# aubin-tchoi/shot-fpfh

Measured on AMD Instinct MI355X. Metric: descriptors/sec (SHOT+FPFH) on 1M-pt cloud, higher is better.
Workload: dtype f64

## Files before the change

### shot_fpfh_amd/csrc/common.h

```cpp
#pragma once
#include <hip/hip_runtime.h>

#include <cstdarg>
#include <cstdint>
#include <cstdio>
#include <cstring>
#include <map>
#include <atomic>
#include <tuple>
#include <string>
#include <vector>

#include "../../include/shotfpfh.h"

extern std::atomic<unsigned long long> g_sf_sync_count;
static inline hipError_t sf_counted_stream_sync(hipStream_t s)
{
    g_sf_sync_count.fetch_add(1, std::memory_order_relaxed);
    return hipStreamSynchronize(s);
}
#define hipStreamSynchronize(s) sf_counted_stream_sync(s)

#define SF_WAVE 64
constexpr double SF_DBL_MAX = 1.7976931348623157e308;
// ... 12 lines not shown
#define SF_HIP_NULL(call)                                                                             \
    do {                                                                                              \
        hipError_t e_ = (call);                                                                       \
        if (e_ != hipSuccess) {                                                                       \
            sf_set_error("%s failed: %s (%s:%d)", #call, hipGetErrorString(e_), __FILE__, __LINE__); \
            return nullptr;                                                                           \
        }                                                                                             \
    } while (0)

#define SF_CHECK(expr)      \
    do {                    \
        int rc_ = (expr);   \
        if (rc_ != SF_OK) return rc_; \
    } while (0)

struct sf_prof_entry {
    int64_t launches = 0;
    std::vector<std::pair<hipEvent_t, hipEvent_t>> pending;
    double total_ms = 0.0;
};

struct sf_graph {
    hipGraph_t graph = nullptr;
    hipGraphExec_t exec = nullptr;
    std::vector<void *> held;
};

struct sf_ctx {
    int device = 0;
    hipStream_t stream = nullptr;
    hipStream_t streams[2] = {nullptr, nullptr};
    hipEvent_t join_event = nullptr;
    hipEvent_t mark_event = nullptr;
    bool profiling = false;
    std::string prof_only;
    std::map<std::string, sf_prof_entry> prof;
    std::vector<hipEvent_t> event_pool;
    void *comm = nullptr;
    int nranks = 1, rank = 0;
    bool collective_stats = false;
    void *scratch = nullptr;
    size_t scratch_bytes = 0;
    void *pinned = nullptr;
    double *shot_coef = nullptr;
    volatile int *dev_flag = nullptr;
    std::multimap<size_t, void *> pool_free;
    std::map<void *, size_t> pool_size;
    size_t pool_cached = 0;
    sf_graph *capture = nullptr;
};

int sf_pool_alloc(sf_ctx *ctx, size_t bytes, void **out);
void sf_pool_release(sf_ctx *ctx, void *p);
void sf_pool_trim(sf_ctx *ctx);
template <typename T>
static inline int sf_palloc(sf_ctx *ctx, T **out, size_t count)
{
    void *p = nullptr;
    int rc = sf_pool_alloc(ctx, (count ? count : 1) * sizeof(T), &p);
    *out = (T *)p;
    return rc;
}

struct sf_pool_guard {
    sf_ctx *ctx;
    std::vector<void *> held;
// ... 53 lines not shown
            ctx->prof[name].launches++;
        }
    }
};

#define SF_LAUNCH(ctx, name, kernel, grid, block, ...)                                   \
    do {                                                                                 \
        sf_launch_timer t_((ctx), (name));                                               \
        hipLaunchKernelGGL(kernel, (grid), (block), 0, (ctx)->stream, __VA_ARGS__);      \
    } while (0);                                                                         \
    SF_HIP(hipGetLastError())

struct sf_cloud {
    int64_t n = 0;
    double *xyz_orig = nullptr;
    double *nrm_orig = nullptr;
    int32_t *zperm = nullptr;
    int32_t *perm_int = nullptr;
    bool bbox_known = false;
    double bbox_lo[3] = {0, 0, 0}, bbox_hi[3] = {0, 0, 0};
    uint64_t grid_gen = 0;
    double cell = 0.0;
    double inv_cell = 0.0;
    double lo[3] = {0, 0, 0};
    int dim[3] = {1, 1, 1};
    int xsub = 1;
    int64_t ncell = 0;
    int32_t *cell_start = nullptr;
    int32_t *perm = nullptr;
    int32_t *inv_perm = nullptr;
    bool inv_perm_valid = false;
    double *xs = nullptr, *ys = nullptr, *zs = nullptr;
    double *rec = nullptr;
    bool normals_sorted = false;
    double nrm_max2 = -1.0;
    int64_t pop_begin = 0, pop_end = 0;
    double *z_orig = nullptr;
    std::vector<double> z_host;
    int32_t *cell_count = nullptr;
    int64_t cell_count_cap = 0;
    bool count_dirty = false;
    std::vector<int64_t> layer_first;
    std::map<std::pair<double, bool>, std::pair<double, int64_t>> list_stats;
    struct search_record {
        int64_t total = 0, n_overflow = 0, ovf_total = 0, cap = 0, hist[5] = {0, 0, 0, 0, 0};
        int32_t max_count = 0, max_count_all = 0;
        bool folded = false;
    };
    typedef std::tuple<double, double, int, int64_t, int64_t> search_key;
    std::map<search_key, search_record> search_records;
};

struct sf_nbrs {
    int64_t m = 0;
    double radius = 0.0;
    int64_t total = 0;
    int64_t max_count = 0;
    int64_t max_count_all = 0;
    bool view = false;
    bool self = false;
    int64_t self_begin = 0;
    double *qx = nullptr, *qy = nullptr, *qz = nullptr;
    int32_t *qrow = nullptr;
    int32_t *count = nullptr;
    int64_t *offset = nullptr;
    int32_t *idx = nullptr;
    int32_t *idx_ovf = nullptr;
    int64_t cap = 0;
    int64_t n_overflow = 0;
    int64_t hist[5] = {0, 0, 0, 0, 0};
    bool planned = false;
    int main_chunks = 4;
    int tail_limit = 0x7fffffff;
    int32_t *tail_sel = nullptr;
    int64_t n_tail = 0;
    int32_t *mid_sel = nullptr;
    int64_t n_mid = 0;
    int64_t view_first = 0;
    uint64_t grid_gen = 0;
};

static inline void sf_nbrs_stamp(sf_nbrs *nb, const sf_cloud *c) { nb->grid_gen = c->grid_gen; }
static inline int sf_nbrs_on_grid(const sf_nbrs *nb, const sf_cloud *c, const char *who)
{
// ... 58 lines not shown
```

### shot_fpfh_amd/csrc/context.hip

```cpp
#include "common.h"

static thread_local char g_err[1024] = "";

void sf_set_error(const char *fmt, ...)
{
    va_list ap;
    va_start(ap, fmt);
    vsnprintf(g_err, sizeof(g_err), fmt, ap);
    va_end(ap);
}

extern "C" const char *sf_last_error(void) { return g_err; }
#ifndef SF_BUILD_ID
#define SF_BUILD_ID "unknown"
#endif
extern "C" const char *sf_version(void) { return "shotfpfh-gfx950 0.3 build " SF_BUILD_ID; }

extern "C" int sf_device_count(void)
{
    int n = 0;
    if (hipGetDeviceCount(&n) != hipSuccess) return 0;
    return n;
}

extern "C" sf_ctx *sf_create(int device)
{
    int n = 0;
    hipError_t e = hipGetDeviceCount(&n);
    if (e != hipSuccess || n <= 0) {
        sf_set_error("no HIP device available (%s); libshotfpfh has no CPU fallback",
                     e == hipSuccess ? "device count 0" : hipGetErrorString(e));
        return nullptr;
    }
    if (device < 0 || device >= n) {
        sf_set_error("device %d out of range (0..%d)", device, n - 1);
        return nullptr;
    }
    SF_HIP_NULL(hipSetDevice(device));
    sf_ctx *ctx = new sf_ctx();
    ctx->device = device;
    e = hipStreamCreateWithFlags(&ctx->streams[0], hipStreamNonBlocking);
    int prio_lo = 0, prio_hi = 0;
    (void)hipDeviceGetStreamPriorityRange(&prio_lo, &prio_hi);
    if (e == hipSuccess) e = hipStreamCreateWithPriority(&ctx->streams[1], hipStreamNonBlocking, prio_hi);
    if (e == hipSuccess) e = hipEventCreateWithFlags(&ctx->join_event, hipEventDisableTiming);
    if (e == hipSuccess) e = hipEventCreateWithFlags(&ctx->mark_event, hipEventDisableTiming);
    if (e != hipSuccess) {
        sf_set_error("hipStreamCreate failed: %s", hipGetErrorString(e));
        delete ctx;
        return nullptr;
    }
    ctx->stream = ctx->streams[0];
    void *flag = nullptr;
    if (hipHostMalloc(&flag, 64, hipHostMallocMapped) != hipSuccess) {
        sf_set_error("hipHostMalloc failed");
        delete ctx;
        return nullptr;
    }
    memset(flag, 0, 64);
    ctx->dev_flag = (volatile int *)flag;
    return ctx;
}

int sf_ctx_check_flag(sf_ctx *ctx)
{
    if (!ctx->dev_flag || !*ctx->dev_flag) return SF_OK;
    const int bits = *ctx->dev_flag;
    *ctx->dev_flag = 0;
    sf_set_error("an index array passed to the library holds values out of range:%s%s (the offending elements were skipped)",
                 bits & SF_FLAG_ROWS_GATHER ? " sf_rows_gather's row selection" : "",
                 bits & SF_FLAG_VOXEL_ORDER ? " sf_voxels_select's visiting order" : "");
    return SF_ERR_ARG;
}

extern "C" void sf_destroy(sf_ctx *ctx)
{
    if (!ctx) return;
    (void)hipSetDevice(ctx->device);
    (void)hipStreamSynchronize(ctx->streams[0]);
    (void)hipStreamSynchronize(ctx->streams[1]);
    ctx->stream = ctx->streams[0];
    sf_comm_destroy(ctx);
    for (auto &kv : ctx->prof)
        for (auto &p : kv.second.pending) {
            ctx->event_pool.push_back(p.first);
            ctx->event_pool.push_back(p.second);
        }
    for (hipEvent_t ev : ctx->event_pool) (void)hipEventDestroy(ev);
    if (ctx->scratch) (void)hipFree(ctx->scratch);
    if (ctx->pinned) (void)hipHostFree(ctx->pinned);
    if (ctx->shot_coef) (void)hipFree(ctx->shot_coef);
    if (ctx->dev_flag) (void)hipHostFree((void *)ctx->dev_flag);
    sf_pool_trim(ctx);
    for (auto &kv : ctx->pool_size) (void)hipFree(kv.first);
    (void)hipEventDestroy(ctx->join_event);
    (void)hipStreamDestroy(ctx->streams[0]);
    (void)hipStreamDestroy(ctx->streams[1]);
    delete ctx;
}

extern "C" int sf_sync(sf_ctx *ctx)
{
    if (!ctx) { sf_set_error("null ctx"); return SF_ERR_ARG; }
    SF_HIP(hipStreamSynchronize(ctx->streams[0]));
    SF_HIP(hipStreamSynchronize(ctx->streams[1]));
    return sf_ctx_check_flag(ctx);
}

extern "C" int sf_fork(sf_ctx *ctx)
{
    if (!ctx) { sf_set_error("null ctx"); return SF_ERR_ARG; }
    if (ctx->stream != ctx->streams[0]) { sf_set_error("sf_fork: already forked"); return SF_ERR_STATE; }
    SF_HIP(hipEventRecord(ctx->join_event, ctx->streams[0]));
    SF_HIP(hipStreamWaitEvent(ctx->streams[1], ctx->join_event, 0));
    ctx->stream = ctx->streams[1];
    return SF_OK;
}

extern "C" int sf_switch(sf_ctx *ctx, int side)
{
    if (!ctx || side < 0 || side > 1) { sf_set_error("sf_switch: bad argument"); return SF_ERR_ARG; }
    ctx->stream = ctx->streams[side];
    return SF_OK;
}

extern "C" int sf_join(sf_ctx *ctx)
{
    if (!ctx) { sf_set_error("null ctx"); return SF_ERR_ARG; }
    SF_HIP(hipEventRecord(ctx->join_event, ctx->streams[1]));
    SF_HIP(hipStreamWaitEvent(ctx->streams[0], ctx->join_event, 0));
    ctx->stream = ctx->streams[0];
    return SF_OK;
}

extern "C" int sf_mark(sf_ctx *ctx)
{
    if (!ctx) { sf_set_error("null ctx"); return SF_ERR_ARG; }
    SF_HIP(hipEventRecord(ctx->mark_event, ctx->stream));
    return SF_OK;
}

extern "C" int sf_wait_mark(sf_ctx *ctx)
{
    if (!ctx) { sf_set_error("null ctx"); return SF_ERR_ARG; }
    SF_HIP(hipStreamWaitEvent(ctx->stream, ctx->mark_event, 0));
    return SF_OK;
}

extern "C" void *sf_stream(sf_ctx *ctx) { return ctx ? (void *)ctx->stream : nullptr; }

std::atomic<unsigned long long> g_sf_sync_count{0};
extern "C" unsigned long long sf_sync_count(void) { return g_sf_sync_count.load(std::memory_order_relaxed); }

extern "C" int sf_graph_begin(sf_ctx *ctx)
{
    if (!ctx) { sf_set_error("null ctx"); return SF_ERR_ARG; }
    if (ctx->capture) { sf_set_error("sf_graph_begin: already capturing"); return SF_ERR_STATE; }
    if (ctx->stream != ctx->streams[0]) { sf_set_error("sf_graph_begin: forked (sf_join first)"); return SF_ERR_STATE; }
    if (ctx->profiling) { sf_set_error("sf_graph_begin: launch timers are on (sf_profile(0) first)"); return SF_ERR_STATE; }
    SF_HIP(hipSetDevice(ctx->device));
    SF_HIP(hipStreamSynchronize(ctx->streams[0]));
    SF_HIP(hipStreamSynchronize(ctx->streams[1]));
    SF_HIP(hipStreamBeginCapture(ctx->streams[0], hipStreamCaptureModeThreadLocal));
    ctx->capture = new sf_graph();
    return SF_OK;
}

extern "C" sf_graph *sf_graph_end(sf_ctx *ctx)
{
    if (!ctx || !ctx->capture) { sf_set_error("sf_graph_end: not capturing"); return nullptr; }
    sf_graph *g = ctx->capture;
    ctx->capture = nullptr;
    ctx->stream = ctx->streams[0];
    hipError_t e = hipStreamEndCapture(ctx->streams[0], &g->graph);
    if (e == hipSuccess && g->graph) e = hipGraphInstantiate(&g->exec, g->graph, nullptr, nullptr, 0);
    if (e != hipSuccess || !g->exec) {
        sf_set_error("sf_graph_end: the step could not be captured (%s)", hipGetErrorString(e));
        (void)hipGetLastError();
        sf_graph_free(ctx, g);
        return nullptr;
    }
    return g;
}

extern "C" int sf_graph_launch(sf_ctx *ctx, sf_graph *g)
{
    if (!ctx || !g || !g->exec) { sf_set_error("sf_graph_launch: bad argument"); return SF_ERR_ARG; }
    if (ctx->capture) { sf_set_error("sf_graph_launch: capturing"); return SF_ERR_STATE; }
    SF_HIP(hipGraphLaunch(g->exec, ctx->streams[0]));
    return SF_OK;
}

extern "C" void sf_graph_free(sf_ctx *ctx, sf_graph *g)
{
    if (!g) return;
// ... 212 lines not shown
```

### shot_fpfh_amd/csrc/fpfh.hip

```cpp
#include <algorithm>
#include <cmath>
#include <cstring>

#include "common.h"
#include "device_util.h"

namespace {

#include "fpfh_mc.h"

template <typename CT, int LPR, int NP, int NCH>
__global__ __launch_bounds__(256) void k_fpfh(const double *__restrict__ rec, const int64_t *__restrict__ offset,
                                              const int32_t *__restrict__ cnt, const int32_t *__restrict__ idx,
                                              int64_t nbrs_begin,
                                              const int32_t *__restrict__ kp_pos, int64_t m, int nb3, int stride,
                                              const CT *__restrict__ counts, unsigned table_bytes,
                                              const int32_t *__restrict__ kk, double *__restrict__ out)
{
    constexpr int BPP = 16 / (int)sizeof(CT);
    constexpr int RPI = 64 / LPR;
    const int lane = threadIdx.x & 63;
    const int64_t q = sf_uniform64(sf_xcd_block() * 4 + (threadIdx.x >> 6));
    if (q >= m) return;
    const int64_t i = kp_pos ? (int64_t)kp_pos[q] : nbrs_begin + q;
// ... 464 lines not shown
}

static int fpfh_run(sf_ctx *ctx, sf_cloud *c, sf_nbrs *nb, sf_spfh *sp, const int64_t *kp_idx, int64_t m, double *out, int flags,
                    double *cov);

extern "C" int sf_fpfh(sf_ctx *ctx, sf_cloud *c, sf_nbrs *nb, sf_spfh *sp, const int64_t *kp_idx, int64_t m, double *out,
                       int flags)
{
    return fpfh_run(ctx, c, nb, sp, kp_idx, m, out, flags, nullptr);
}

extern "C" int sf_fpfh_moments(sf_ctx *ctx, sf_cloud *c, sf_nbrs *nb, sf_spfh *sp, int64_t m, double *out, double *cov_dev, int flags)
{
    if (!cov_dev) { sf_set_error("sf_fpfh_moments: null cov"); return SF_ERR_ARG; }
    if (nb && sp && !fpfh_mc_carries_moments(nb, sp)) {
        sf_set_error("sf_fpfh_moments: these lists / this table do not take a K7 form that carries the frame moments");
        return SF_ERR_UNSUPPORTED;
    }
    return fpfh_run(ctx, c, nb, sp, nullptr, m, out, flags, cov_dev);
}

static int fpfh_run(sf_ctx *ctx, sf_cloud *c, sf_nbrs *nb, sf_spfh *sp, const int64_t *kp_idx, int64_t m, double *out, int flags,
                    double *cov)
{
    if (!ctx || !c || !nb || !sp || !out || m < 0) { sf_set_error("sf_fpfh: bad argument"); return SF_ERR_ARG; }
    if (!nb->self) { sf_set_error("sf_fpfh: needs a sf_radius_search_self result"); return SF_ERR_ARG; }
    SF_CHECK(sf_nbrs_on_grid(nb, c, "sf_fpfh"));
    if (!kp_idx && m != nb->m) { sf_set_error("sf_fpfh: m must equal the query count when kp_idx is NULL"); return SF_ERR_ARG; }
    if (kp_idx && !(nb->self_begin == 0 && nb->m == c->n)) {
        sf_set_error("sf_fpfh: keypoints by index need neighbour lists of the whole cloud");
        return SF_ERR_ARG;
    }
    SF_HIP(hipSetDevice(ctx->device));
    sf_pool_guard tmp(ctx);
    int32_t *pos = nullptr;
    if (kp_idx && m) {
        const int64_t *src = kp_idx;
        int64_t *dkp = nullptr;
        int *dbad = nullptr;
        if (!(flags & SF_IN_DEVICE)) {
            SF_CHECK(tmp.alloc(&dkp, (size_t)m));
            SF_HIP(hipMemcpyAsync(dkp, kp_idx, (size_t)m * sizeof(int64_t), hipMemcpyHostToDevice, ctx->stream));
            src = dkp;
        }
        SF_CHECK(tmp.alloc(&pos, (size_t)m));
        SF_CHECK(tmp.alloc(&dbad, 1));
        SF_HIP(hipMemsetAsync(dbad, 0, sizeof(int), ctx->stream));
        SF_CHECK(sf_cloud_ensure_inv_perm(ctx, c));
        SF_LAUNCH(ctx, "k7_map_positions", k_map_positions, dim3((unsigned)sf_div_up(m, 256)), dim3(256), src,
                  c->inv_perm, m, c->n, pos, dbad);
        int bad = 0;
        SF_HIP(hipMemcpyAsync(&bad, dbad, sizeof(int), hipMemcpyDeviceToHost, ctx->stream));
        SF_HIP(hipStreamSynchronize(ctx->stream));
        if (bad) {
            sf_set_error("sf_fpfh: keypoint index out of range for a cloud of %lld points", (long long)c->n);
            return SF_ERR_ARG;
        }
    }
    const int64_t tot = m * sp->nb3;
    double *dout = out, *owned = nullptr;
    if (!(flags & SF_OUT_DEVICE)) {
        SF_CHECK(tmp.alloc(&owned, (size_t)tot));
        dout = owned;
    }
    int rc = SF_OK;
    if (m && sp->n_bins > SF_FAST_FPFH_BINS && sp->elem_bytes != 1) {
// ... 15 lines not shown
```

### shot_fpfh_amd/csrc/grid.hip

```cpp
#include <rocprim/device/device_radix_sort.hpp>
#include <rocprim/device/device_reduce.hpp>
#include <rocprim/device/device_scan.hpp>
#include <rocprim/iterator/transform_iterator.hpp>

#include <algorithm>
#include <cmath>

#include <cstring>

#include "common.h"
#include "device_util.h"

#ifndef SF_SORT_BITS
#define SF_SORT_BITS 10
#endif
#ifndef SF_SORT_BLOCK
#define SF_SORT_BLOCK 1024
#endif
#ifndef SF_SORT_ITEMS
#define SF_SORT_ITEMS 6
#endif
using sf_onesweep = rocprim::radix_sort_onesweep_config<rocprim::kernel_config<SF_SORT_BLOCK, SF_SORT_ITEMS>, rocprim::kernel_config<SF_SORT_BLOCK, SF_SORT_ITEMS>,
                                                        SF_SORT_BITS, rocprim::block_radix_rank_algorithm::match>;
using sf_sort_config = rocprim::radix_sort_config<rocprim::default_config, rocprim::default_config, sf_onesweep, 65536>;
// ... 77 lines not shown
    if (i >= n) return;
    const int64_t o = zperm[i];
    dst[3 * i + 0] = src[3 * o + 0];
    dst[3 * i + 1] = src[3 * o + 1];
    dst[3 * i + 2] = src[3 * o + 2];
}

__global__ __launch_bounds__(256) void k_layer_bounds(const double *__restrict__ z, int64_t n, double lo, double inv_cell, int nlayers,
                                                      int64_t *__restrict__ first)
{
    const int lane = threadIdx.x & 63;
    const int l = blockIdx.x * 4 + (threadIdx.x >> 6);
    if (l > nlayers) return;
    int64_t a = 0, b = n;
    while (b - a > 64) {
        const int64_t step = (b - a + 63) / 64;
        const int64_t i = a + (int64_t)lane * step;
        const bool below = i < b && sf_cell_coord(z[i], lo, inv_cell, nlayers) < l;
        const int k = __popcll(__ballot(below));
        if (k == 0) { b = a; break; }
        const int64_t na = a + (int64_t)(k - 1) * step + 1;
        const int64_t nb = k < 64 ? a + (int64_t)k * step : b;
        a = na;
        b = nb < b ? nb : b;
    }
    if (b > a) {
        const int64_t i = a + lane;
        const bool below = i < b && sf_cell_coord(z[i], lo, inv_cell, nlayers) < l;
        a += __popcll(__ballot(below));
    }
    if (lane == 0) first[l] = l == nlayers ? n : a;
}

__global__ void k_gather_sorted(const double *__restrict__ xyz, const double *__restrict__ nrm, const int32_t *__restrict__ perm_int,
                                const int32_t *__restrict__ zperm, int32_t *__restrict__ perm,
                                int64_t base, int64_t n, double *__restrict__ xs, double *__restrict__ ys,
                                double *__restrict__ zs, double *__restrict__ rec, unsigned *__restrict__ zero_word)
{
    int64_t i = (int64_t)blockIdx.x * blockDim.x + threadIdx.x;
    if (i == 0 && zero_word) *zero_word = 0u;
    if (i >= n) return;
    i += base;
    int64_t o = perm_int[i];
    perm[i] = zperm[o];
    const double x = xyz[3 * o + 0], y = xyz[3 * o + 1], z = xyz[3 * o + 2];
    xs[i] = x; ys[i] = y; zs[i] = z;
    rec[6 * i + 0] = x; rec[6 * i + 1] = y; rec[6 * i + 2] = z;
    if (nrm) {
        rec[6 * i + 3] = nrm[3 * o + 0];
        rec[6 * i + 4] = nrm[3 * o + 1];
        rec[6 * i + 5] = nrm[3 * o + 2];
    }
}

__global__ void k_inv_perm(const int32_t *__restrict__ perm, int64_t base, int64_t n, int32_t *__restrict__ inv_perm)
{
    int64_t i = (int64_t)blockIdx.x * blockDim.x + threadIdx.x;
    if (i >= n) return;
    i += base;
    inv_perm[perm[i]] = (int32_t)i;
}

__global__ void k_gather_normals(const double *__restrict__ nrm, const int32_t *__restrict__ perm, int64_t base, int64_t n,
                                 double *__restrict__ rec)
{
    int64_t i = (int64_t)blockIdx.x * blockDim.x + threadIdx.x;
    if (i >= n) return;
    i += base;
    int64_t o = perm[i];
    rec[6 * i + 3] = nrm[3 * o + 0];
    rec[6 * i + 4] = nrm[3 * o + 1];
    rec[6 * i + 5] = nrm[3 * o + 2];
}

#define SF_LONG_GAP 65536
struct sf_gap { int64_t lo, len; int32_t val, pad; };
__global__ __launch_bounds__(256) void k_cell_start(const int32_t *__restrict__ sorted_cid, int64_t cid_base, int64_t base, int64_t n,
                                                    int64_t ncell, int32_t *__restrict__ cell_start, sf_gap *__restrict__ gaps,
                                                    unsigned *__restrict__ n_gaps)
{
    const int lane = threadIdx.x & 63;
    const int64_t i = (int64_t)blockIdx.x * blockDim.x + threadIdx.x;
    int64_t lo = 0, len = 0;
    if (i <= n) {
// ... 116 lines not shown
                unsigned long long s;
                do {
                    s = j >= 0 ? __hip_atomic_load(&st[j], __ATOMIC_RELAXED, __HIP_MEMORY_SCOPE_AGENT) : SF_SCAN_PREFIX;
                } while (__ballot((s >> 62) == 0ull));
                const unsigned long long have = __ballot((s >> 62) == 2ull);
                const int stop = have ? __builtin_ctzll(have) : 64;
                int val = lane <= stop ? (int)(unsigned)(s & 0xffffffffull) : 0;
#pragma unroll
                for (int off = 32; off > 0; off >>= 1) val += __shfl_xor(val, off);
                excl += val;
                if (have) break;
            }
            if (lane == 0) __hip_atomic_store(&st[t], SF_SCAN_PREFIX | (unsigned long long)(unsigned)(excl + total), __ATOMIC_RELAXED, __HIP_MEMORY_SCOPE_AGENT);
        }
        if (lane == 0) s_prefix = excl;
    }
    __syncthreads();
    const int add = base + s_prefix + before;
#pragma unroll
    for (int k = 0; k < SF_SCAN_ITEMS; ++k)
        if (k < left) p[k] = add + v[k];
}

__global__ void k_cell_place(const int32_t *__restrict__ cid, const int32_t *__restrict__ place, const int32_t *__restrict__ start_rel,
                             int64_t first, int64_t n, int2 *__restrict__ slot)
{
    const int64_t i = (int64_t)blockIdx.x * blockDim.x + threadIdx.x;
    if (i >= n) return;
    const int c = cid[i];
    slot[(int64_t)start_rel[c] + place[i] - first] = make_int2((int)(first + i), c);
}

__global__ void k_cell_settle(const int2 *__restrict__ slot, const int32_t *__restrict__ start_rel, const double *__restrict__ xyz,
                              const double *__restrict__ nrm, const int32_t *__restrict__ zperm, int32_t *__restrict__ perm,
                              int32_t *__restrict__ perm_int, int64_t base, int64_t n, double *__restrict__ xs, double *__restrict__ ys,
                              double *__restrict__ zs, double *__restrict__ rec)
{
    const int64_t p = (int64_t)blockIdx.x * blockDim.x + threadIdx.x;
    if (p >= n) return;
    const int2 me = slot[p];
    const int64_t cs = (int64_t)start_rel[me.y] - base, ce = (int64_t)start_rel[me.y + 1] - base;
    int r = 0;
    for (int64_t j = cs; j < ce; ++j) r += slot[j].x < me.x ? 1 : 0;
    const int64_t i = base + cs + r, o = me.x;
    perm_int[i] = me.x;
    perm[i] = zperm[o];
    const double x = xyz[3 * o + 0], y = xyz[3 * o + 1], z = xyz[3 * o + 2];
    xs[i] = x; ys[i] = y; zs[i] = z;
    rec[6 * i + 0] = x; rec[6 * i + 1] = y; rec[6 * i + 2] = z;
    if (nrm) {
        rec[6 * i + 3] = nrm[3 * o + 0];
        rec[6 * i + 4] = nrm[3 * o + 1];
        rec[6 * i + 5] = nrm[3 * o + 2];
    }
}

__global__ void k_layer_first(const int32_t *__restrict__ cell_start, int64_t layer_cells, int nl, int64_t *__restrict__ out)
{
    const int z = blockIdx.x * blockDim.x + threadIdx.x;
    if (z <= nl) out[z] = cell_start[(int64_t)z * layer_cells];
}

}

static void cloud_release_grid(sf_ctx *ctx, sf_cloud *c)
{
    void *ptrs[] = {c->cell_start, c->perm, c->perm_int, c->inv_perm, c->xs, c->ys, c->zs, c->rec};
    for (void *p : ptrs)
        if (p) {
            if (ctx) sf_pool_release(ctx, p); else (void)hipFree(p);
        }
    c->cell_start = c->perm = c->perm_int = c->inv_perm = nullptr;
    c->inv_perm_valid = false;
    c->xs = c->ys = c->zs = c->rec = nullptr;
    c->normals_sorted = false;
    c->cell = 0.0;
    c->pop_begin = c->pop_end = 0;
    c->layer_first.clear();
}

static int upload_in_zorder(sf_ctx *ctx, sf_cloud *c, const double *src, int flags, double *dst)
{
    const int64_t n = c->n;
    if (!n) return SF_OK;
    sf_pool_guard tmp(ctx);
    const double *dsrc = src;
    if (!(flags & SF_IN_DEVICE)) {
        double *stage = nullptr;
        SF_CHECK(tmp.alloc(&stage, (size_t)n * 3));
        SF_HIP(hipMemcpyAsync(stage, src, (size_t)n * 24, hipMemcpyHostToDevice, ctx->stream));
        dsrc = stage;
    }
    SF_LAUNCH(ctx, "k0_upload", k_upload_gather, dim3((unsigned)sf_div_up(n, 256)), dim3(256), dsrc, (const int32_t *)c->zperm, n, dst);
    SF_HIP(hipStreamSynchronize(ctx->stream));
    return SF_OK;
}

static int cloud_upload(sf_ctx *ctx, sf_cloud *c, const double *xyz, const double *normals, int flags)
{
// ... 26 lines not shown
        }
        SF_LAUNCH(ctx, "k0_upload", k_upload_gather, dim3((unsigned)sf_div_up(n, 256)), dim3(256), dsrc, (const int32_t *)c->zperm, n,
                  c->xyz_orig);
        SF_HIP(hipStreamSynchronize(ctx->stream));
    }
    if (normals) {
        SF_CHECK(sf_pool_alloc(ctx, bytes, (void **)&c->nrm_orig));
        SF_CHECK(upload_in_zorder(ctx, c, normals, flags, c->nrm_orig));
    }
    return SF_OK;
}

extern "C" sf_cloud *sf_cloud_upload(sf_ctx *ctx, const double *xyz, const double *normals, int64_t n, int flags)
{
    if (!ctx || (!xyz && n > 0) || n < 0 || n > 2147483000LL) {
        sf_set_error("sf_cloud_upload: bad arguments (n=%lld)", (long long)n);
        return nullptr;
    }
    SF_HIP_NULL(hipSetDevice(ctx->device));
    sf_cloud *c = new sf_cloud();
    c->n = n;
    if (cloud_upload(ctx, c, xyz, normals, flags) != SF_OK) {
        sf_cloud_free(ctx, c);
        return nullptr;
    }
    return c;
}

extern "C" int sf_cloud_set_normals(sf_ctx *ctx, sf_cloud *c, const double *normals, int flags)
{
    if (!ctx || !c || !normals) { sf_set_error("sf_cloud_set_normals: null argument"); return SF_ERR_ARG; }
    SF_HIP(hipSetDevice(ctx->device));
    size_t bytes = (size_t)(c->n ? c->n : 1) * 24;
    if (!c->nrm_orig) SF_CHECK(sf_pool_alloc(ctx, bytes, (void **)&c->nrm_orig));
    SF_CHECK(upload_in_zorder(ctx, c, normals, flags, c->nrm_orig));
    c->normals_sorted = false;
    c->nrm_max2 = -1.0;
    return SF_OK;
}

namespace {
__global__ void k_normals_max2(const double *__restrict__ nrm, int64_t n, unsigned long long *__restrict__ out)
{
    double mx = 0.0;
    for (int64_t i = (int64_t)blockIdx.x * blockDim.x + threadIdx.x; i < n; i += (int64_t)gridDim.x * blockDim.x) {
        const double a = nrm[3 * i], b = nrm[3 * i + 1], c = nrm[3 * i + 2];
        const double v = (a * a + b * b) + c * c;
        mx = v <= 1.7976931348623157e308 ? fmax(mx, v) : INFINITY;
    }
    for (int off = 32; off > 0; off >>= 1) mx = fmax(mx, __shfl_xor(mx, off));
    if ((threadIdx.x & 63) == 0) atomicMax(out, (unsigned long long)__double_as_longlong(mx));
}
}

int sf_cloud_normals_max2(sf_ctx *ctx, sf_cloud *c, double *out)
{
    if (!c->nrm_orig) { sf_set_error("this operation needs normals, but the cloud has none"); return SF_ERR_STATE; }
    if (c->nrm_max2 < 0.0) {
        sf_pool_guard tmp(ctx);
        unsigned long long *d = nullptr;
        void *pin = nullptr;
        SF_CHECK(tmp.alloc(&d, (size_t)1));
        SF_CHECK(sf_ctx_pinned(ctx, &pin));
        SF_HIP(hipMemsetAsync(d, 0, sizeof(unsigned long long), ctx->stream));
        if (c->n) SF_LAUNCH(ctx, "k1_normals_max", k_normals_max2, dim3(512), dim3(256), (const double *)c->nrm_orig, c->n, d);
        SF_HIP(hipMemcpyAsync(pin, d, sizeof(unsigned long long), hipMemcpyDeviceToHost, ctx->stream));
        SF_HIP(hipStreamSynchronize(ctx->stream));
        long long bits = *(const long long *)pin;
        double v;
        static_assert(sizeof(v) == sizeof(bits), "");
        memcpy(&v, &bits, sizeof(v));
        c->nrm_max2 = v;
    }
    *out = c->nrm_max2;
    return SF_OK;
}

int sf_cloud_ensure_inv_perm(sf_ctx *ctx, sf_cloud *c)
{
    if (c->inv_perm_valid) return SF_OK;
    if (!c->perm || !c->inv_perm) { sf_set_error("grid not built"); return SF_ERR_STATE; }
    const int64_t np = c->pop_end - c->pop_begin;
    if (np > 0)
        SF_LAUNCH(ctx, "k1_inv_perm", k_inv_perm, dim3((unsigned)sf_div_up(np, 256)), dim3(256), (const int32_t *)c->perm,
                  c->pop_begin, np, c->inv_perm);
    c->inv_perm_valid = true;
    return SF_OK;
}

int sf_cloud_ensure_sorted_normals(sf_ctx *ctx, sf_cloud *c)
{
    if (c->normals_sorted) return SF_OK;
    if (!c->nrm_orig) { sf_set_error("this operation needs normals, but the cloud has none"); return SF_ERR_STATE; }
    if (!c->perm) { sf_set_error("grid not built"); return SF_ERR_STATE; }
    const int64_t np = c->pop_end - c->pop_begin;
    if (np > 0) {
        SF_LAUNCH(ctx, "k1_gather_normals", k_gather_normals, dim3((unsigned)sf_div_up(np, 256)), dim3(256),
                  c->nrm_orig, c->perm_int, c->pop_begin, np, c->rec);
        hipStream_t other = ctx->stream == ctx->streams[0] ? ctx->streams[1] : ctx->streams[0];
        SF_HIP(hipEventRecord(ctx->join_event, ctx->stream));
        SF_HIP(hipStreamWaitEvent(other, ctx->join_event, 0));
    }
    c->normals_sorted = true;
    return SF_OK;
}

int sf_cloud_bbox_raw(sf_ctx *ctx, const double *xyz_dev, int64_t n, double lo[3], double hi[3])
{
    for (int a = 0; a < 3; ++a) lo[a] = hi[a] = 0.0;
    if (!n) return SF_OK;
    const int nb = 1024;
    void *scr = nullptr;
    SF_CHECK(sf_ctx_scratch(ctx, ((size_t)nb * 6 + 8) * sizeof(double), &scr));
    SF_LAUNCH(ctx, "k1_bbox", k_bbox_partial, dim3(nb), dim3(256), xyz_dev, n, (double *)scr);
    double *fin = (double *)scr + (size_t)nb * 6;
    SF_LAUNCH(ctx, "k1_bbox", k_bbox_final, dim3(1), dim3(384), (const double *)scr, nb, fin);
    void *pin = nullptr;
    SF_CHECK(sf_ctx_pinned(ctx, &pin));
    double *part = (double *)pin;
    SF_HIP(hipMemcpyAsync(part, fin, 6 * sizeof(double), hipMemcpyDeviceToHost, ctx->stream));
    SF_HIP(hipStreamSynchronize(ctx->stream));
    for (int a = 0; a < 3; ++a) { lo[a] = part[a]; hi[a] = part[3 + a]; }
    for (int a = 0; a < 3; ++a)
        if (!std::isfinite(lo[a]) || !std::isfinite(hi[a])) {
// ... 131 lines not shown
    c->normals_sorted = c->nrm_orig != nullptr;
    const bool force_radix = getenv("SF_K1_RADIX") != nullptr;
    if (ns > 0 && !force_radix && slab_cells <= SF_COUNT_CELLS_PER_POINT * ns && ns <= 64 * slab_cells) {
        const int64_t slab_tiles = sf_div_up(slab_cells, (int64_t)SF_SCAN_TILE), n_status = slab_tiles + 1;
        const int64_t fill_blocks = sf_div_up(ncell + 1 - slab_cells, (int64_t)SF_SCAN_TILE);
        int32_t *cid = nullptr, *place = nullptr;
        int2 *slot = nullptr;
        unsigned long long *status = nullptr;
        SF_CHECK(tmp.alloc(&cid, (size_t)ns));
        SF_CHECK(tmp.alloc(&place, (size_t)ns));
        SF_CHECK(tmp.alloc(&slot, (size_t)ns));
        SF_CHECK(tmp.alloc(&status, (size_t)n_status));
        int32_t *start_rel = c->cell_start + cid_base;
        if (hipPeekAtLastError() != hipSuccess) c->count_dirty = true;
        if (c->cell_count_cap < slab_cells || c->count_dirty) {
            if (c->cell_count_cap < slab_cells) {
                if (c->cell_count) sf_pool_release(ctx, c->cell_count);
                c->cell_count = nullptr;
                c->cell_count_cap = 0;
                SF_CHECK(sf_pool_alloc(ctx, (size_t)slab_cells * sizeof(int32_t), (void **)&c->cell_count));
                c->cell_count_cap = slab_cells;
            }
            sf_launch_timer t_(ctx, "k1_cell_zero");
            SF_HIP(hipMemsetAsync(c->cell_count, 0, (size_t)c->cell_count_cap * sizeof(int32_t), ctx->stream));
        }
        c->count_dirty = true;
        SF_LAUNCH(ctx, "k1_cell_count", k_cell_count, dim3((unsigned)sf_div_up(std::max(ns, n_status), 256)), dim3(256), c->xyz_orig, base, ns, g,
                  (int)cid_base, c->cell_count, cid, place, status, n_status);
        SF_LAUNCH(ctx, "k1_cell_scan", k_cell_scan, dim3((unsigned)(slab_tiles + fill_blocks)), dim3(SF_SCAN_TPB), c->cell_count, c->cell_start, ncell,
                  cid_base, slab_cells, slab_tiles, (int32_t)base, (int32_t)ns, status);
        c->count_dirty = false;
        SF_LAUNCH(ctx, "k1_cell_place", k_cell_place, dim3((unsigned)sf_div_up(ns, 256)), dim3(256), (const int32_t *)cid,
                  (const int32_t *)place, (const int32_t *)start_rel, base, ns, slot);
        SF_LAUNCH(ctx, "k1_cell_settle", k_cell_settle, dim3((unsigned)sf_div_up(ns, 256)), dim3(256), (const int2 *)slot,
                  (const int32_t *)start_rel, c->xyz_orig, (const double *)c->nrm_orig, (const int32_t *)c->zperm, c->perm, c->perm_int, base, ns,
                  c->xs, c->ys, c->zs, c->rec);
        return SF_OK;
    }
    int32_t *key_in = nullptr, *val_in = nullptr, *cid_sorted = nullptr;
    SF_CHECK(tmp.alloc(&cid_sorted, (size_t)std::max<int64_t>(ns, 1)));
    if (ns > 0) {
        SF_CHECK(tmp.alloc(&key_in, (size_t)ns + 1));
        SF_CHECK(tmp.alloc(&val_in, (size_t)ns + 1));
        SF_LAUNCH(ctx, "k1_cell_ids", k_cell_ids, dim3((unsigned)sf_div_up(ns, 256)), dim3(256), c->xyz_orig, base, ns, g, key_in, val_in,
                  (int)cid_base);
    }
    sf_gap *gaps = nullptr;
    unsigned *n_gaps = nullptr;
    SF_CHECK(tmp.alloc(&gaps, (size_t)(ncell / SF_LONG_GAP + 2)));
    SF_CHECK(tmp.alloc(&n_gaps, 1));
    if (ns > 0) {
        size_t tmp_bytes = 0;
        SF_HIP(sort_cells(nullptr, tmp_bytes, key_in, cid_sorted, val_in, c->perm_int + base, (size_t)ns, bits, ctx->stream));
        char *stmp = nullptr;
        SF_CHECK(tmp.alloc(&stmp, tmp_bytes ? tmp_bytes : 8));
        {
            sf_launch_timer t_(ctx, "k1_radix_sort");
            SF_HIP(sort_cells(stmp, tmp_bytes, key_in, cid_sorted, val_in, c->perm_int + base, (size_t)ns, bits, ctx->stream));
        }
        SF_LAUNCH(ctx, "k1_gather_sorted", k_gather_sorted, dim3((unsigned)sf_div_up(ns, 256)), dim3(256), c->xyz_orig,
                  (const double *)c->nrm_orig, (const int32_t *)c->perm_int, (const int32_t *)c->zperm, c->perm, base, ns, c->xs, c->ys, c->zs,
                  c->rec, n_gaps);
    }
    {
        if (ns <= 0) SF_HIP(hipMemsetAsync(n_gaps, 0, sizeof(unsigned), ctx->stream));
        SF_LAUNCH(ctx, "k1_cell_start", k_cell_start, dim3((unsigned)sf_div_up(ns + 1, 256)), dim3(256), cid_sorted, cid_base, base, ns,
                  ncell, c->cell_start, gaps, n_gaps);
        SF_LAUNCH(ctx, "k1_cell_fill_long", k_cell_fill_long, dim3(1024), dim3(256), (const sf_gap *)gaps, (const unsigned *)n_gaps,
                  c->cell_start);
    }
    return SF_OK;
}

static int cloud_layer_first(sf_ctx *ctx, sf_cloud *c)
{
    if (!c->cell_start) { sf_set_error("grid not built"); return SF_ERR_STATE; }
    const int nl = c->dim[2];
    if ((int64_t)c->layer_first.size() == (int64_t)nl + 1) return SF_OK;
    sf_pool_guard tmp(ctx);
    int64_t *d = nullptr;
    SF_CHECK(tmp.alloc(&d, (size_t)nl + 1));
    SF_LAUNCH(ctx, "k1_layer_first", k_layer_first, dim3((unsigned)sf_div_up(nl + 1, 256)), dim3(256), (const int32_t *)c->cell_start,
              (int64_t)c->dim[0] * c->dim[1], nl, d);
    c->layer_first.assign((size_t)nl + 1, 0);
    SF_HIP(hipMemcpyAsync(c->layer_first.data(), d, ((size_t)nl + 1) * sizeof(int64_t), hipMemcpyDeviceToHost, ctx->stream));
    SF_HIP(hipStreamSynchronize(ctx->stream));
    return SF_OK;
}

extern "C" int sf_cloud_layer_table(sf_ctx *ctx, sf_cloud *c, int64_t *first, int64_t cap, int64_t *n_layers)
{
    if (!ctx || !c || !n_layers) { sf_set_error("sf_cloud_layer_table: null argument"); return SF_ERR_ARG; }
    SF_CHECK(cloud_layer_first(ctx, c));
    *n_layers = c->dim[2];
    if (first) {
// ... 70 lines not shown
```

### shot_fpfh_amd/csrc/host_stage.h

```cpp
#pragma once
#include "common.h"

static inline int check_nbrs(sf_ctx *ctx, sf_cloud *c, sf_nbrs *nb, const char *who)
{
    if (!ctx || !c || !nb) { sf_set_error("%s: null argument", who); return SF_ERR_ARG; }
    if (!c->xs) { sf_set_error("%s: grid not built", who); return SF_ERR_STATE; }
    SF_CHECK(sf_nbrs_on_grid(nb, c, who));
    SF_HIP(hipSetDevice(ctx->device));
    return SF_OK;
}

static inline int stage_in(sf_pool_guard &g, const double *src, size_t count, int flags, const double **dev)
{
    if (!src) { *dev = nullptr; return SF_OK; }
    if (flags & SF_IN_DEVICE) { *dev = src; return SF_OK; }
    double *owned = nullptr;
    SF_CHECK(g.alloc(&owned, count));
    if (count) SF_HIP(hipMemcpyAsync(owned, src, count * sizeof(double), hipMemcpyHostToDevice, g.ctx->stream));
    *dev = owned;
    return SF_OK;
}

static inline int stage_out(sf_pool_guard &g, double *dst, size_t count, int flags, double **dev)
{
    if (flags & SF_OUT_DEVICE) { *dev = dst; return SF_OK; }
    return g.alloc(dev, count);
}

static inline int finish_out(sf_ctx *ctx, double *dst, size_t count, int flags, const double *dev)
{
    if (!(flags & SF_OUT_DEVICE) && count)
        SF_HIP(hipMemcpyAsync(dst, dev, count * sizeof(double), hipMemcpyDeviceToHost, ctx->stream));
    return SF_OK;
}

static inline int stage_sync(sf_ctx *ctx, int flags)
{
    if ((flags & (SF_IN_DEVICE | SF_OUT_DEVICE)) != (SF_IN_DEVICE | SF_OUT_DEVICE)) SF_HIP(hipStreamSynchronize(ctx->stream));
    return SF_OK;
}


// ... 1 lines not shown
```

### shot_fpfh_amd/csrc/icp.hip

```cpp
#include "common.h"
#include "device_util.h"
#include "select.h"

namespace {

constexpr int ICP_BLOCKS = 256;
constexpr int ICP_NV = 32;

__global__ void k_transform(const double *__restrict__ pts, const int64_t *__restrict__ sel, int64_t m,
                            const double *__restrict__ Rt, double *__restrict__ out)
{
    const int64_t i = (int64_t)blockIdx.x * blockDim.x + threadIdx.x;
    if (i >= m) return;
    const int64_t j = sel ? sel[i] : i;
    const double x = pts[3 * j], y = pts[3 * j + 1], z = pts[3 * j + 2];
    double ox = x, oy = y, oz = z;
    if (Rt) {
        ox = ((x * Rt[0] + y * Rt[1]) + z * Rt[2]) + Rt[9];
        oy = ((x * Rt[3] + y * Rt[4]) + z * Rt[5]) + Rt[10];
        oz = ((x * Rt[6] + y * Rt[7]) + z * Rt[8]) + Rt[11];
    }
    out[3 * i] = ox; out[3 * i + 1] = oy; out[3 * i + 2] = oz;
}

// ... 231 lines not shown
    if (!ctx || !pts_dev || !Rt || n < 0) { sf_set_error("sf_transform_points: bad argument"); return SF_ERR_ARG; }
    SF_HIP(hipSetDevice(ctx->device));
    if (!n) return SF_OK;
    sf_pool_guard tmp(ctx);
    double *dRt = nullptr;
    SF_CHECK(tmp.alloc(&dRt, 12));
    SF_HIP(hipMemcpyAsync(dRt, Rt, 12 * sizeof(double), hipMemcpyHostToDevice, ctx->stream));
    SF_LAUNCH(ctx, "i0_transform", k_transform, dim3((unsigned)sf_div_up(n, 256)), dim3(256), (const double *)pts_dev,
              (const int64_t *)nullptr, n, (const double *)dRt, pts_dev);
    SF_HIP(hipStreamSynchronize(ctx->stream));
    return SF_OK;
}

static int icp_chain(const char *who, sf_ctx *ctx, sf_cloud *ref, const double *pts_dev, const double *nrm_dev, const int64_t *sel_dev,
                     int64_t m, const double *Rt, double d_max, int mode, double epsilon, int loss, double scale, double *sums,
                     double trim = 1.0)
{
    if (ref->n < 1) { sf_set_error("%s: empty reference cloud", who); return SF_ERR_ARG; }
    sf_pool_guard tmp(ctx);
    double *dRt = nullptr, *moved = nullptr, *partial = nullptr, *dout = nullptr, *dmean = nullptr;
    if (Rt) {
        SF_CHECK(tmp.alloc(&dRt, 12));
        SF_HIP(hipMemcpyAsync(dRt, Rt, 12 * sizeof(double), hipMemcpyHostToDevice, ctx->stream));
    }
    SF_CHECK(tmp.alloc(&moved, (size_t)m * 3));
    SF_CHECK(tmp.alloc(&partial, (size_t)ICP_BLOCKS * ICP_NV));
    SF_CHECK(tmp.alloc(&dout, 80));
    SF_CHECK(tmp.alloc(&dmean, 8));
    SF_LAUNCH(ctx, "i0_transform", k_transform, dim3((unsigned)sf_div_up(m, 256)), dim3(256), pts_dev, sel_dev, m,
              (const double *)dRt, moved);
    sf_nbrs *nb = sf_knn_search(ctx, ref, moved, m, 1, SF_IN_DEVICE);
    if (!nb) return SF_ERR_HIP;
    struct nb_guard { sf_ctx *c; sf_nbrs *n; ~nb_guard() { sf_nbrs_free(c, n); } } nbg{ctx, nb};
    if (mode != 0) SF_CHECK(sf_cloud_ensure_sorted_normals(ctx, ref));
    SF_HIP(hipMemsetAsync(dout, 0, 48 * sizeof(double), ctx->stream));
    const dim3 grid(ICP_BLOCKS), block(256);
    const int32_t *qrow = (const int32_t *)nb->qrow;
    const double *no_mean = nullptr, *cut = nullptr;
    const bool trimmed = trim < 1.0;
    if (trimmed) {
        uint64_t *keys = nullptr;
        SF_CHECK(tmp.alloc(&keys, (size_t)m));
#define SF_ICP_KEYS(MODE)                                                                                                            \
    SF_LAUNCH(ctx, "i2_icp_keys", (k_icp_keys<MODE>), grid, block, nb->qx, nb->qy, nb->qz, nb->idx, qrow, ref->rec, nrm_dev, sel_dev, \
              (const double *)dRt, m, d_max, epsilon, keys)
        if (mode == 0) { SF_ICP_KEYS(0); }
        else if (mode == 1) { SF_ICP_KEYS(1); }
        else if (mode == 2) { SF_ICP_KEYS(2); }
        else { SF_ICP_KEYS(3); }
#undef SF_ICP_KEYS
        SF_CHECK(sf_select_launch(ctx, keys, m, 0, trim, dout + 48));
        cut = dout + 48;
    }
#define SF_ICP_PASS(PASS, MODE, mean)                                                                                                \
    SF_LAUNCH(ctx, "i1_icp_sums", (k_icp_sums<PASS, MODE>), grid, block, nb->qx, nb->qy, nb->qz, nb->idx, qrow, ref->rec, nrm_dev,    \
              sel_dev, (const double *)dRt, m, d_max, epsilon, loss, scale, mean, cut, partial)
    if (mode == 0) { SF_ICP_PASS(0, 0, no_mean); }
    else if (mode == 1) { SF_ICP_PASS(0, 1, no_mean); }
    else if (mode == 2) { SF_ICP_PASS(0, 2, no_mean); }
    else { SF_ICP_PASS(0, 3, no_mean); }
    SF_LAUNCH(ctx, "i1_icp_means", k_icp_means, dim3(1), dim3(64), (const double *)partial, ICP_BLOCKS, dout, dmean);
    if (mode == 0) { SF_ICP_PASS(1, 0, (const double *)dmean); }
    else if (mode == 1) { SF_ICP_PASS(1, 1, no_mean); }
    else if (mode == 2) { SF_ICP_PASS(1, 2, no_mean); }
    else { SF_ICP_PASS(1, 3, no_mean); }
#undef SF_ICP_PASS
// ... 112 lines not shown
```

Before: 584.1 million.

## Split cell-record packing into its own kernel with optional side-stream overlap

Moves construction of the interleaved 6-double cell record array out of the gather and settle kernels into a separate kernel. The new kernel stages records in shared memory so the writes are coalesced `double2` stores. It can optionally run on the secondary stream, with a lazy event join before any consumer of `rec` (FPFH, SHOT stages, ICP, normals). Gather and settle kernels also switch to an XCD-aware block mapping. The overlap path is only enabled when `SF_K1_NO_OVERLAP` is set to 0. By default the records kernel runs serially, which adds a launch and re-reads xs/ys/zs in exchange for cleaner stores.

Result: no change. 586.2 million (median of 6 runs) (+0.4%).

```diff
diff --git a/shot_fpfh_amd/csrc/common.h b/shot_fpfh_amd/csrc/common.h
--- a/shot_fpfh_amd/csrc/common.h
+++ b/shot_fpfh_amd/csrc/common.h
@@ -68,6 +68,8 @@
     hipStream_t streams[2] = {nullptr, nullptr};
     hipEvent_t join_event = nullptr;
     hipEvent_t mark_event = nullptr;
+    hipEvent_t records_event = nullptr;
+    uint64_t records_issued = 0, records_joined = 0;
     bool profiling = false;
     std::string prof_only;
     std::map<std::string, sf_prof_entry> prof;
@@ -187,6 +189,7 @@
     bool inv_perm_valid = false;
     double *xs = nullptr, *ys = nullptr, *zs = nullptr;
     double *rec = nullptr;
+    uint64_t records_pending = 0;
     bool normals_sorted = false;
     double nrm_max2 = -1.0;
     int64_t pop_begin = 0, pop_end = 0;
@@ -205,6 +208,9 @@
     typedef std::tuple<double, double, int, int64_t, int64_t> search_key;
     std::map<search_key, search_record> search_records;
 };
+
+int sf_cloud_join_records(sf_ctx *ctx, sf_cloud *c);
+static inline int sf_cloud_ensure_records(sf_ctx *ctx, sf_cloud *c) { return c->records_pending ? sf_cloud_join_records(ctx, c) : SF_OK; }
 
 struct sf_nbrs {
     int64_t m = 0;
diff --git a/shot_fpfh_amd/csrc/context.hip b/shot_fpfh_amd/csrc/context.hip
--- a/shot_fpfh_amd/csrc/context.hip
+++ b/shot_fpfh_amd/csrc/context.hip
@@ -45,6 +45,7 @@
     if (e == hipSuccess) e = hipStreamCreateWithPriority(&ctx->streams[1], hipStreamNonBlocking, prio_hi);
     if (e == hipSuccess) e = hipEventCreateWithFlags(&ctx->join_event, hipEventDisableTiming);
     if (e == hipSuccess) e = hipEventCreateWithFlags(&ctx->mark_event, hipEventDisableTiming);
+    if (e == hipSuccess) e = hipEventCreateWithFlags(&ctx->records_event, hipEventDisableTiming);
     if (e != hipSuccess) {
         sf_set_error("hipStreamCreate failed: %s", hipGetErrorString(e));
         delete ctx;
@@ -94,6 +95,7 @@
     sf_pool_trim(ctx);
     for (auto &kv : ctx->pool_size) (void)hipFree(kv.first);
     (void)hipEventDestroy(ctx->join_event);
+    (void)hipEventDestroy(ctx->records_event);
     (void)hipStreamDestroy(ctx->streams[0]);
     (void)hipStreamDestroy(ctx->streams[1]);
     delete ctx;
@@ -104,6 +106,7 @@
     if (!ctx) { sf_set_error("null ctx"); return SF_ERR_ARG; }
     SF_HIP(hipStreamSynchronize(ctx->streams[0]));
     SF_HIP(hipStreamSynchronize(ctx->streams[1]));
+    ctx->records_joined = ctx->records_issued;
     return sf_ctx_check_flag(ctx);
 }
 
@@ -161,6 +164,7 @@
     SF_HIP(hipSetDevice(ctx->device));
     SF_HIP(hipStreamSynchronize(ctx->streams[0]));
     SF_HIP(hipStreamSynchronize(ctx->streams[1]));
+    ctx->records_joined = ctx->records_issued;
     SF_HIP(hipStreamBeginCapture(ctx->streams[0], hipStreamCaptureModeThreadLocal));
     ctx->capture = new sf_graph();
     return SF_OK;
diff --git a/shot_fpfh_amd/csrc/fpfh.hip b/shot_fpfh_amd/csrc/fpfh.hip
--- a/shot_fpfh_amd/csrc/fpfh.hip
+++ b/shot_fpfh_amd/csrc/fpfh.hip
@@ -520,6 +520,7 @@
         return SF_ERR_ARG;
     }
     SF_HIP(hipSetDevice(ctx->device));
+    SF_CHECK(sf_cloud_ensure_records(ctx, c));
     sf_pool_guard tmp(ctx);
     int32_t *pos = nullptr;
     if (kp_idx && m) {
diff --git a/shot_fpfh_amd/csrc/grid.hip b/shot_fpfh_amd/csrc/grid.hip
--- a/shot_fpfh_amd/csrc/grid.hip
+++ b/shot_fpfh_amd/csrc/grid.hip
@@ -133,24 +133,48 @@
     if (lane == 0) first[l] = l == nlayers ? n : a;
 }
 
-__global__ void k_gather_sorted(const double *__restrict__ xyz, const double *__restrict__ nrm, const int32_t *__restrict__ perm_int,
+__global__ void k_gather_sorted(const double *__restrict__ xyz, const int32_t *__restrict__ perm_int,
                                 const int32_t *__restrict__ zperm, int32_t *__restrict__ perm,
                                 int64_t base, int64_t n, double *__restrict__ xs, double *__restrict__ ys,
-                                double *__restrict__ zs, double *__restrict__ rec, unsigned *__restrict__ zero_word)
-{
-    int64_t i = (int64_t)blockIdx.x * blockDim.x + threadIdx.x;
+                                double *__restrict__ zs, unsigned *__restrict__ zero_word)
+{
+    int64_t i = sf_xcd_block() * blockDim.x + threadIdx.x;
     if (i == 0 && zero_word) *zero_word = 0u;
     if (i >= n) return;
     i += base;
     int64_t o = perm_int[i];
     perm[i] = zperm[o];
-    const double x = xyz[3 * o + 0], y = xyz[3 * o + 1], z = xyz[3 * o + 2];
-    xs[i] = x; ys[i] = y; zs[i] = z;
-    rec[6 * i + 0] = x; rec[6 * i + 1] = y; rec[6 * i + 2] = z;
-    if (nrm) {
-        rec[6 * i + 3] = nrm[3 * o + 0];
-        rec[6 * i + 4] = nrm[3 * o + 1];
-        rec[6 * i + 5] = nrm[3 * o + 2];
+    xs[i] = xyz[3 * o + 0]; ys[i] = xyz[3 * o + 1]; zs[i] = xyz[3 * o + 2];
+}
+
+#define SF_REC_TPB 256
+__global__ __launch_bounds__(SF_REC_TPB) void k_cell_records(const double *__restrict__ xs, const double *__restrict__ ys,
+                                                             const double *__restrict__ zs, const double *__restrict__ nrm,
+                                                             const int32_t *__restrict__ perm_int, int64_t base, int64_t n,
+                                                             double *__restrict__ rec)
+{
+    __shared__ double2 s_rec[SF_REC_TPB / 64][3 * 64];
+    const int lane = threadIdx.x & 63, w = threadIdx.x >> 6;
+    const int64_t w0 = (sf_xcd_block() * (SF_REC_TPB / 64) + w) * 64;
+    const int64_t left = n - w0;
+    if (lane < left) {
+        const int64_t i = base + w0 + lane;
+        double nx = 0.0, ny = 0.0, nz = 0.0;
+        if (nrm) {
+            const int64_t o = perm_int[i];
+            nx = nrm[3 * o + 0]; ny = nrm[3 * o + 1]; nz = nrm[3 * o + 2];
+        }
+        s_rec[w][3 * lane + 0] = make_double2(xs[i], ys[i]);
+        s_rec[w][3 * lane + 1] = make_double2(zs[i], nx);
+        s_rec[w][3 * lane + 2] = make_double2(ny, nz);
+    }
+    __syncthreads();
+    double2 *out = reinterpret_cast<double2 *>(rec + 6 * (base + w0));
+    const int64_t chunks = 3 * (left < 64 ? left : 64);
+#pragma unroll
+    for (int k = 0; k < 3; ++k) {
+        const int c = k * 64 + lane;
+        if (c < chunks) out[c] = s_rec[w][c];
     }
 }
 
@@ -333,11 +357,11 @@
 }
 
 __global__ void k_cell_settle(const int2 *__restrict__ slot, const int32_t *__restrict__ start_rel, const double *__restrict__ xyz,
-                              const double *__restrict__ nrm, const int32_t *__restrict__ zperm, int32_t *__restrict__ perm,
+                              const int32_t *__restrict__ zperm, int32_t *__restrict__ perm,
                               int32_t *__restrict__ perm_int, int64_t base, int64_t n, double *__restrict__ xs, double *__restrict__ ys,
-                              double *__restrict__ zs, double *__restrict__ rec)
-{
-    const int64_t p = (int64_t)blockIdx.x * blockDim.x + threadIdx.x;
+                              double *__restrict__ zs)
+{
+    const int64_t p = sf_xcd_block() * blockDim.x + threadIdx.x;
     if (p >= n) return;
     const int2 me = slot[p];
     const int64_t cs = (int64_t)start_rel[me.y] - base, ce = (int64_t)start_rel[me.y + 1] - base;
@@ -346,14 +370,7 @@
     const int64_t i = base + cs + r, o = me.x;
     perm_int[i] = me.x;
     perm[i] = zperm[o];
-    const double x = xyz[3 * o + 0], y = xyz[3 * o + 1], z = xyz[3 * o + 2];
-    xs[i] = x; ys[i] = y; zs[i] = z;
-    rec[6 * i + 0] = x; rec[6 * i + 1] = y; rec[6 * i + 2] = z;
-    if (nrm) {
-        rec[6 * i + 3] = nrm[3 * o + 0];
-        rec[6 * i + 4] = nrm[3 * o + 1];
-        rec[6 * i + 5] = nrm[3 * o + 2];
-    }
+    xs[i] = xyz[3 * o + 0]; ys[i] = xyz[3 * o + 1]; zs[i] = xyz[3 * o + 2];
 }
 
 __global__ void k_layer_first(const int32_t *__restrict__ cell_start, int64_t layer_cells, int nl, int64_t *__restrict__ out)
@@ -364,8 +381,46 @@
 
 }
 
+int sf_cloud_join_records(sf_ctx *ctx, sf_cloud *c)
+{
+    if (c->records_pending > ctx->records_joined) {
+        SF_HIP(hipStreamWaitEvent(ctx->streams[0], ctx->records_event, 0));
+        ctx->records_joined = ctx->records_issued;
+    }
+    c->records_pending = 0;
+    return SF_OK;
+}
+
+static int launch_records(sf_ctx *ctx, sf_cloud *c, int64_t base, int64_t ns)
+{
+    const char *sw = getenv("SF_K1_NO_OVERLAP");
+    const bool beside = ctx->stream == ctx->streams[0] && !ctx->capture && sw && *sw && atoi(sw) == 0;
+    struct on_stream {
+        sf_ctx *ctx;
+        hipStream_t keep;
+        on_stream(sf_ctx *x, hipStream_t s) : ctx(x), keep(x->stream) { x->stream = s; }
+        ~on_stream() { ctx->stream = keep; }
+    };
+    if (beside) {
+        SF_HIP(hipEventRecord(ctx->join_event, ctx->streams[0]));
+        SF_HIP(hipStreamWaitEvent(ctx->streams[1], ctx->join_event, 0));
+    }
+    {
+        on_stream side(ctx, beside ? ctx->streams[1] : ctx->stream);
+        SF_LAUNCH(ctx, "k1_cell_records", k_cell_records, dim3(sf_xcd_grid(sf_div_up(ns, SF_REC_TPB))), dim3(SF_REC_TPB), (const double *)c->xs,
+                  (const double *)c->ys, (const double *)c->zs, (const double *)c->nrm_orig, (const int32_t *)c->perm_int, base, ns, c->rec);
+    }
+    if (beside) {
+        SF_HIP(hipEventRecord(ctx->records_event, ctx->streams[1]));
+        c->records_pending = ++ctx->records_issued;
+    }
+    return SF_OK;
+}
+
 static void cloud_release_grid(sf_ctx *ctx, sf_cloud *c)
 {
+    if (ctx) (void)sf_cloud_ensure_records(ctx, c);
+    c->records_pending = 0;
     void *ptrs[] = {c->cell_start, c->perm, c->perm_int, c->inv_perm, c->xs, c->ys, c->zs, c->rec};
     for (void *p : ptrs)
         if (p) {
@@ -458,6 +513,7 @@
     if (!ctx || !c || !normals) { sf_set_error("sf_cloud_set_normals: null argument"); return SF_ERR_ARG; }
     SF_HIP(hipSetDevice(ctx->device));
     size_t bytes = (size_t)(c->n ? c->n : 1) * 24;
+    SF_CHECK(sf_cloud_ensure_records(ctx, c));
     if (!c->nrm_orig) SF_CHECK(sf_pool_alloc(ctx, bytes, (void **)&c->nrm_orig));
     SF_CHECK(upload_in_zorder(ctx, c, normals, flags, c->nrm_orig));
     c->normals_sorted = false;
@@ -516,6 +572,7 @@
 
 int sf_cloud_ensure_sorted_normals(sf_ctx *ctx, sf_cloud *c)
 {
+    SF_CHECK(sf_cloud_ensure_records(ctx, c));
     if (c->normals_sorted) return SF_OK;
     if (!c->nrm_orig) { sf_set_error("this operation needs normals, but the cloud has none"); return SF_ERR_STATE; }
     if (!c->perm) { sf_set_error("grid not built"); return SF_ERR_STATE; }
@@ -713,10 +770,9 @@
         c->count_dirty = false;
         SF_LAUNCH(ctx, "k1_cell_place", k_cell_place, dim3((unsigned)sf_div_up(ns, 256)), dim3(256), (const int32_t *)cid,
                   (const int32_t *)place, (const int32_t *)start_rel, base, ns, slot);
-        SF_LAUNCH(ctx, "k1_cell_settle", k_cell_settle, dim3((unsigned)sf_div_up(ns, 256)), dim3(256), (const int2 *)slot,
-                  (const int32_t *)start_rel, c->xyz_orig, (const double *)c->nrm_orig, (const int32_t *)c->zperm, c->perm, c->perm_int, base, ns,
-                  c->xs, c->ys, c->zs, c->rec);
-        return SF_OK;
+        SF_LAUNCH(ctx, "k1_cell_settle", k_cell_settle, dim3(sf_xcd_grid(sf_div_up(ns, 256))), dim3(256), (const int2 *)slot,
+                  (const int32_t *)start_rel, c->xyz_orig, (const int32_t *)c->zperm, c->perm, c->perm_int, base, ns, c->xs, c->ys, c->zs);
+        return launch_records(ctx, c, base, ns);
     }
     int32_t *key_in = nullptr, *val_in = nullptr, *cid_sorted = nullptr;
     SF_CHECK(tmp.alloc(&cid_sorted, (size_t)std::max<int64_t>(ns, 1)));
@@ -739,9 +795,9 @@
             sf_launch_timer t_(ctx, "k1_radix_sort");
             SF_HIP(sort_cells(stmp, tmp_bytes, key_in, cid_sorted, val_in, c->perm_int + base, (size_t)ns, bits, ctx->stream));
         }
-        SF_LAUNCH(ctx, "k1_gather_sorted", k_gather_sorted, dim3((unsigned)sf_div_up(ns, 256)), dim3(256), c->xyz_orig,
-                  (const double *)c->nrm_orig, (const int32_t *)c->perm_int, (const int32_t *)c->zperm, c->perm, base, ns, c->xs, c->ys, c->zs,
-                  c->rec, n_gaps);
+        SF_LAUNCH(ctx, "k1_gather_sorted", k_gather_sorted, dim3(sf_xcd_grid(sf_div_up(ns, 256))), dim3(256), c->xyz_orig,
+                  (const int32_t *)c->perm_int, (const int32_t *)c->zperm, c->perm, base, ns, c->xs, c->ys, c->zs, n_gaps);
+        SF_CHECK(launch_records(ctx, c, base, ns));
     }
     {
         if (ns <= 0) SF_HIP(hipMemsetAsync(n_gaps, 0, sizeof(unsigned), ctx->stream));
diff --git a/shot_fpfh_amd/csrc/host_stage.h b/shot_fpfh_amd/csrc/host_stage.h
--- a/shot_fpfh_amd/csrc/host_stage.h
+++ b/shot_fpfh_amd/csrc/host_stage.h
@@ -7,7 +7,7 @@
     if (!c->xs) { sf_set_error("%s: grid not built", who); return SF_ERR_STATE; }
     SF_CHECK(sf_nbrs_on_grid(nb, c, who));
     SF_HIP(hipSetDevice(ctx->device));
-    return SF_OK;
+    return sf_cloud_ensure_records(ctx, c);
 }
 
 static inline int stage_in(sf_pool_guard &g, const double *src, size_t count, int flags, const double **dev)
diff --git a/shot_fpfh_amd/csrc/icp.hip b/shot_fpfh_amd/csrc/icp.hip
--- a/shot_fpfh_amd/csrc/icp.hip
+++ b/shot_fpfh_amd/csrc/icp.hip
@@ -287,6 +287,7 @@
     sf_nbrs *nb = sf_knn_search(ctx, ref, moved, m, 1, SF_IN_DEVICE);
     if (!nb) return SF_ERR_HIP;
     struct nb_guard { sf_ctx *c; sf_nbrs *n; ~nb_guard() { sf_nbrs_free(c, n); } } nbg{ctx, nb};
+    SF_CHECK(sf_cloud_ensure_records(ctx, ref));
     if (mode != 0) SF_CHECK(sf_cloud_ensure_sorted_normals(ctx, ref));
     SF_HIP(hipMemsetAsync(dout, 0, 48 * sizeof(double), ctx->stream));
     const dim3 grid(ICP_BLOCKS), block(256);
```
